# YoshuaNava/icpslam

Measured on AMD Instinct MI355X. Metric: icp_iterations_per_sec, higher is better.
Workload: dtype f32

## Files before the change

### icpslam_amd/csrc/icp_grid.hip

```cpp
#include <math.h>

#include <cstdlib>
#include <cstring>

#include "icp_env.h"
#include "icp_device.h"
#include "icp_grid_device.h"
#include "icp_kernels.h"

namespace icpgpu {
namespace {

__device__ __forceinline__ int enc_float(float f) {
  const int i = __float_as_int(f);
  return i >= 0 ? i : i ^ 0x7FFFFFFF;
}
inline float dec_float(int e) {
  const int i = e >= 0 ? e : e ^ 0x7FFFFFFF;
  float f;
  std::memcpy(&f, &i, 4);
  return f;
}

__global__ void bbox_init_kernel(int* mm) {
  if (threadIdx.x < 3) mm[threadIdx.x] = 0x7FFFFFFF;
  else if (threadIdx.x < 6) mm[threadIdx.x] = (int)0x80000000;
}

__global__ __launch_bounds__(256) void bbox_kernel(const float4* __restrict__ pts, int n, int* __restrict__ mm) {
  int lo[3] = {0x7FFFFFFF, 0x7FFFFFFF, 0x7FFFFFFF}, hi[3] = {(int)0x80000000, (int)0x80000000, (int)0x80000000};
  for (int i = blockIdx.x * 256 + threadIdx.x; i < n; i += gridDim.x * 256) {
    const float4 p = pts[i];
    if (finite3(p.x, p.y, p.z)) {
      const int e[3] = {enc_float(p.x), enc_float(p.y), enc_float(p.z)};
#pragma unroll
      for (int a = 0; a < 3; ++a) {
        lo[a] = min(lo[a], e[a]);
        hi[a] = max(hi[a], e[a]);
      }
    }
  }
#pragma unroll
  for (int a = 0; a < 3; ++a) {
#pragma unroll
    for (int off = 32; off > 0; off >>= 1) {
      lo[a] = min(lo[a], __shfl_down(lo[a], off, 64));
      hi[a] = max(hi[a], __shfl_down(hi[a], off, 64));
    }
  }
  __shared__ int wmm[4][6];
  const int lane = threadIdx.x & 63, wave = threadIdx.x >> 6;
  if (lane == 0) {
#pragma unroll
    for (int a = 0; a < 3; ++a) {
// ... 113 lines not shown
  int base = 0, total = 0;
#pragma unroll
  for (int w = 0; w < 16; ++w) {
    if (w < wave) base += wtot[w];
    total += wtot[w];
  }
  if (threadIdx.x == 0) stats[0] = total;
  int run = base + incl - s;
  for (int k = lo; k < hi; ++k) {
    const int v = block_sums[k];
    block_sums[k] = run;
    run += v;
  }
}

__global__ __launch_bounds__(256) void scan_apply_kernel(int* __restrict__ counts, int n, const int* __restrict__ block_sums,
                                                         const int* __restrict__ stats) {
  const int base = blockIdx.x * kScanItems + threadIdx.x * SCAN_PER_THREAD;
  int v[SCAN_PER_THREAD], s = 0;
#pragma unroll
  for (int k = 0; k < SCAN_PER_THREAD; ++k) {
    v[k] = (base + k < n) ? counts[base + k] : 0;
    s += v[k];
  }
  int tot;
  int run = block_exclusive_scan_256(s, &tot) + block_sums[blockIdx.x];
#pragma unroll
  for (int k = 0; k < SCAN_PER_THREAD; ++k) {
    if (base + k < n) counts[base + k] = run;
    run += v[k];
  }
  if (blockIdx.x == 0 && threadIdx.x == 0) counts[n] = stats[0];
}

__global__ __launch_bounds__(256) void grid_scatter_kernel(const float4* __restrict__ pts, int n,
                                                           const int* __restrict__ cell_of_point,
                                                           const int* __restrict__ rank,
                                                           const int* __restrict__ cell_start,
                                                           const int* __restrict__ orig_index,
                                                           float4* __restrict__ sorted) {
  const int i = blockIdx.x * 256 + threadIdx.x;
  if (i >= n) return;
  const int c = cell_of_point[i];
  if (c < 0) return;
  const float4 p = pts[i];
  sorted[cell_start[c] + rank[i]] = make_float4(p.x, p.y, p.z, __int_as_float(orig_index ? orig_index[i] : i));
}

constexpr int WQ_MAX_QPW = 16;

constexpr int WQ_WAVES = 4;
constexpr int WQ_BLOCK = WQ_WAVES * 64;

template <bool WRITE_KEYS, bool FUSE_REDUCE, bool LIST_UNMATCHED, bool PACK_SHORT_ROWS>
__global__ __launch_bounds__(WQ_BLOCK) void nn_wave_kernel(const float4* __restrict__ src, int n_s, int qpw, int xcd_map, Xform T,
                                                           const float4* __restrict__ sorted,
                                                           const int* __restrict__ cell_start, GridDesc g, float accept_thr,
                                                           unsigned long long* __restrict__ keys,
                                                           double* __restrict__ partials, int* __restrict__ unmatched,
                                                           int* __restrict__ unmatched_count) {
  const int lane = threadIdx.x & 63, wave = threadIdx.x >> 6;
  const int lb = xcd_map ? (int)(blockIdx.x & 7u) * (int)(gridDim.x >> 3) + (int)(blockIdx.x >> 3) : (int)blockIdx.x;
  const int k0 = lb * WQ_WAVES + wave, stride = gridDim.x * WQ_WAVES;

  double acc = 0.0;
  int qi = -1, pi = -1;
  if (lane >= 1 && lane <= 3) pi = lane - 1;
  else if (lane >= 4 && lane <= 6) qi = lane - 4;
  else if (lane >= 7 && lane <= 15) { qi = (lane - 7) / 3; pi = (lane - 7) % 3; }
  else if (lane == 16) qi = 3;

  float lpx = 0.f, lpy = 0.f, lpz = 0.f, lmargin = 0.5f;
  int lcx = 0, lcy = 0, lcz = 0, llo = 0, llen = 0;
  bool lfin = false;
  {
    const int sub = lane >> 2, il = k0 + sub * stride;
    if (sub < qpw && il < n_s) {
      const float4 s = src[il];
      xform_point(T, s.x, s.y, s.z, lpx, lpy, lpz);
      lfin = finite3(lpx, lpy, lpz);
      if (lfin) {
        cell_of(g, lpx, lpy, lpz, lcx, lcy, lcz);
        octant_row(cell_start, g, lpx, lpy, lpz, lcx, lcy, lcz, lane & 3, llo, llen, lmargin);
      }
    }
  }
  const unsigned long long fin_mask = __ballot(lfin), row_mask = __ballot(llen > 0);
  const float lsafe = lmargin * g.h * kGridSafety, lsafe_sq = lsafe * lsafe;
  unsigned long long my_key = kEmptyKey;

  for (int qq = 0; qq < qpw; ++qq) {
    const int i = k0 + qq * stride, l0 = qq * 4;
    if (i >= n_s) break;
    LaneBest b{kEmptyKey, 0.f, 0.f, 0.f};
    bool found = false;
    const float px = readlane_f(lpx, l0), py = readlane_f(lpy, l0), pz = readlane_f(lpz, l0);
    if ((fin_mask >> l0) & 1ull) {
      sweep_rows(sorted, llo, llen, row_mask & (0xFull << l0), lane, px, py, pz, b);
      found = merge_lanes(b) && __uint_as_float((unsigned int)(b.key >> 32)) <= readlane_f(lsafe_sq, l0);
      if (!found) {
        const int cx = __builtin_amdgcn_readlane(lcx, l0), cy = __builtin_amdgcn_readlane(lcy, l0),
                  cz = __builtin_amdgcn_readlane(lcz, l0);
        found = grow_cubes<PACK_SHORT_ROWS>(sorted, cell_start, g, px, py, pz, cx, cy, cz, lane, b);
      }
    }
    if constexpr (WRITE_KEYS) {
      if (lane == qq) my_key = found ? b.key : kEmptyKey;
    }
    if constexpr (LIST_UNMATCHED) {
      if (!found && lane == 0) unmatched[atomicAdd(unmatched_count, 1)] = i;
    }
    if constexpr (FUSE_REDUCE) {
      const float d2 = __uint_as_float((unsigned int)(b.key >> 32));
      if (found && d2 <= accept_thr) {
        const double a = qi < 0 ? 1.0 : (qi == 0 ? (double)b.qx : qi == 1 ? (double)b.qy : qi == 2 ? (double)b.qz : (double)d2);
        const double c = pi < 0 ? 1.0 : (pi == 0 ? (double)px : pi == 1 ? (double)py : (double)pz);
        acc += a * c;
      }
    }
  }
  if constexpr (WRITE_KEYS) {
    if (lane < qpw && k0 + lane * stride < n_s) keys[k0 + lane * stride] = my_key;
  }
  if constexpr (FUSE_REDUCE) {
    __shared__ double wterm[WQ_WAVES][kReduceTerms];
    if (lane < kReduceTerms) wterm[wave][lane] = acc;
    __syncthreads();
    if (threadIdx.x < kReduceTerms) {
      double v = 0.0;
#pragma unroll
      for (int w = 0; w < WQ_WAVES; ++w) v += wterm[w][threadIdx.x];
      partials[(size_t)threadIdx.x * gridDim.x + blockIdx.x] = v;
    }
  }
}

template <bool WRITE_KEYS, bool FUSE_REDUCE, bool LIST_UNMATCHED, bool PACK_SHORT_ROWS>
__device__ __forceinline__ void nn_quad_body(const float4* __restrict__ src, int n_s, int qpw, int xcd_map, const Xform& T,
                                             const float4* __restrict__ sorted, const int* __restrict__ cell_start,
                                             const GridDesc& g, float accept_thr, unsigned long long* __restrict__ keys,
                                             double* __restrict__ partials, int* __restrict__ unmatched,
                                             int* __restrict__ unmatched_count, unsigned int* __restrict__ prev_nn, int use_prev,
                                             int cube_start, unsigned long long* __restrict__ count_candidates, int n_blocks,
                                             int bx) {
  const int lane = threadIdx.x & 63, wave = threadIdx.x >> 6;
  const int grp_base = lane & 48, sub = lane & 15;
  unsigned int n_cand = 0;
  const int lb = xcd_map ? (bx & 7) * (n_blocks >> 3) + (bx >> 3) : bx;
  const int k0 = lb * WQ_WAVES + wave, stride = n_blocks * WQ_WAVES;

  double acc = 0.0;
  int cnt = 0;
  int qi = -1, pi = -1;
  if (sub == 0) qi = 3;
  else if (sub <= 3) pi = sub - 1;
  else if (sub <= 6) qi = sub - 4;
  else { qi = (sub - 7) / 3; pi = (sub - 7) % 3; }

  float lpx = 0.f, lpy = 0.f, lpz = 0.f, lmargin = 0.5f;
  int lcx = 0, lcy = 0, lcz = 0, llo = 0, llen = 0;
  bool lfin = false;
  const int il = k0 + (lane >> 2) * stride;
  const bool lvalid = (lane >> 2) < qpw && il < n_s;
  const char* __restrict__ sorted_bytes = reinterpret_cast<const char*>(sorted);
  float lbound = __builtin_nanf("");
  if (lvalid) {
    const float4 s = src[il];
    unsigned int ppos = kNoPrev;
    if (use_prev & 1) ppos = prev_nn[il];
    xform_point(T, s.x, s.y, s.z, lpx, lpy, lpz);
    lfin = finite3(lpx, lpy, lpz);
    if (lfin) {
      cell_of(g, lpx, lpy, lpz, lcx, lcy, lcz);
      if (ppos != kNoPrev) {
        const float4 pq = *reinterpret_cast<const float4*>(sorted_bytes + (size_t)ppos);
        lbound = dist2(pq.x, pq.y, pq.z, lpx, lpy, lpz);
      }
      octant_row_in_ball(cell_start, g, lpx, lpy, lpz, lcx, lcy, lcz, lane & 3, ball_cells_sq(g, lbound), llo, llen, lmargin);
    }
  }
  const unsigned long long fin_mask = __ballot(lfin);
  const float lsafe = lmargin * g.h * kGridSafety, lsafe_sq = lsafe * lsafe;
  const int n_pass = (__popcll(__ballot(lvalid)) + 15) >> 4;

  int slot_of_rank;
  {
    int cand = llen + __builtin_amdgcn_mov_dpp(llen, 0xB1, 0xF, 0xF, true);
    cand += __builtin_amdgcn_mov_dpp(cand, 0x4E, 0xF, 0xF, true);
    const unsigned int mine = ((lvalid ? (unsigned int)cand + 1u : 0u) << 4) | (unsigned int)(lane >> 2);
    int rank = 0;
#pragma unroll
    for (int k = 0; k < 16; ++k) rank += (unsigned int)__builtin_amdgcn_readlane((int)mine, 4 * k) > mine ? 1 : 0;
    slot_of_rank = __builtin_amdgcn_ds_permute((4 * rank + (lane & 3)) << 2, lane >> 2);
  }

  for (int pass = 0; pass < n_pass; ++pass) {
    const int ql = 4 * lane_get_i(slot_of_rank, 4 * (4 * pass + (lane >> 4)));
    const int qi_src = k0 + (ql >> 2) * stride;
    const bool valid = (ql >> 2) < qpw && qi_src < n_s;
    const float px = lane_get_f(lpx, ql), py = lane_get_f(lpy, ql), pz = lane_get_f(lpz, ql);
    const bool fin = (fin_mask >> ql) & 1ull;
    const int lo0 = lane_get_i(llo, ql), lo1 = lane_get_i(llo, ql + 1), lo2 = lane_get_i(llo, ql + 2), lo3 = lane_get_i(llo, ql + 3);
    const int n0 = lane_get_i(llen, ql), n1 = lane_get_i(llen, ql + 1), n2 = lane_get_i(llen, ql + 2), n3 = lane_get_i(llen, ql + 3);
    const int e0 = n0, e1 = e0 + n1, e2 = e1 + n2, L = e2 + n3;
    const unsigned int eb0 = (unsigned int)e0 << 4, eb1 = (unsigned int)e1 << 4, eb2 = (unsigned int)e2 << 4;
    const unsigned int ob0 = (unsigned int)lo0 << 4, ob1 = (unsigned int)(lo1 - e0) << 4, ob2 = (unsigned int)(lo2 - e1) << 4,
                       ob3 = L ? (unsigned int)(lo3 - e2) << 4 : 0u;
    const unsigned int lastb = (unsigned int)max(L - 1, 0) << 4;
    const int l_max = max(max(__builtin_amdgcn_readlane(L, 0), __builtin_amdgcn_readlane(L, 16)),
                          max(__builtin_amdgcn_readlane(L, 32), __builtin_amdgcn_readlane(L, 48)));
    if (count_candidates)
      n_cand += (unsigned int)(__builtin_amdgcn_readlane(L, 0) + __builtin_amdgcn_readlane(L, 16) + __builtin_amdgcn_readlane(L, 32) +
                               __builtin_amdgcn_readlane(L, 48));
    unsigned long long bkey = kEmptyKey;
    unsigned int bpos = 0u;
    unsigned int vb = (unsigned int)sub << 4;
    for (int done = 0; done < l_max; done += 32, vb += 512u) {
      const unsigned int ua = min(vb, lastb), ub = min(vb + 256u, lastb);
      const unsigned int fa = ua + (ua < eb0 ? ob0 : ua < eb1 ? ob1 : ua < eb2 ? ob2 : ob3);
      const unsigned int fb = ub + (ub < eb0 ? ob0 : ub < eb1 ? ob1 : ub < eb2 ? ob2 : ob3);
      const float4 qa = *reinterpret_cast<const float4*>(sorted_bytes + (size_t)fa);
      const float4 qb = *reinterpret_cast<const float4*>(sorted_bytes + (size_t)fb);
      __builtin_amdgcn_sched_barrier(0);
      const unsigned long long ka = ((unsigned long long)__float_as_uint(dist2(qa.x, qa.y, qa.z, px, py, pz)) << 32) | __float_as_uint(qa.w);
      const unsigned long long kb = ((unsigned long long)__float_as_uint(dist2(qb.x, qb.y, qb.z, px, py, pz)) << 32) | __float_as_uint(qb.w);
      if (ka < bkey) { bkey = ka; bpos = fa; }
      if (kb < bkey) { bkey = kb; bpos = fb; }
    }
    const unsigned int dbits = (unsigned int)(bkey >> 32), idx = (unsigned int)bkey;
    const unsigned int dmin = row16_min_u32(dbits);
    const unsigned int imin = row16_min_u32(dbits == dmin ? idx : 0xFFFFFFFFu);
    const unsigned long long win = __ballot(dbits == dmin && idx == imin);
    const int owner = grp_base + __ffs((unsigned int)(win >> grp_base) & 0xFFFFu) - 1;
    unsigned long long gkey = ((unsigned long long)dmin << 32) | imin;
    unsigned int wpos = (unsigned int)lane_get_i((int)bpos, owner);
    bool found = fin && __uint_as_float(dmin) <= lane_get_f(lsafe_sq, ql);

    unsigned long long need = (use_prev & 2) ? 0ull : __ballot(fin && !found && sub == 0);
    while (need) {
      const int gl = __ffsll((long long)need) - 1, sl = __builtin_amdgcn_readlane(ql, gl);
      need &= need - 1;
      const float ux = readlane_f(lpx, sl), uy = readlane_f(lpy, sl), uz = readlane_f(lpz, sl);
      const int cx = __builtin_amdgcn_readlane(lcx, sl), cy = __builtin_amdgcn_readlane(lcy, sl),
                cz = __builtin_amdgcn_readlane(lcz, sl);
      LanePos c{((unsigned long long)(unsigned int)__builtin_amdgcn_readlane((int)(gkey >> 32), gl) << 32) |
                    (unsigned int)__builtin_amdgcn_readlane((int)gkey, gl),
                (unsigned int)__builtin_amdgcn_readlane((int)wpos, gl)};
      const float pb = readlane_f(lbound, sl);
      if (pb < __builtin_inff() && !(__uint_as_float((unsigned int)(c.key >> 32)) <= pb)) {
        c.key = ((unsigned long long)__float_as_uint(pb) << 32) | 0xFFFFFFFFull;
        c.pos = prev_nn[k0 + (sl >> 2) * stride];
      }
      int rho_first = 1;
      {
        const float seed = __uint_as_float((unsigned int)(c.key >> 32));
        const int cap = (use_prev & 1) ? ((cube_start & 1) ? g.r_max : 1) : min((cube_start >> 8) & 0xFF, g.r_max);
        if (seed < __builtin_inff() && cap > 1)
          rho_first = max(1, min((int)ceilf(__builtin_amdgcn_sqrtf(seed) * g.inv_h * (1.0f / kGridSafety)), cap));
      }
      const bool f2 = grow_cubes<PACK_SHORT_ROWS>(sorted, cell_start, g, ux, uy, uz, cx, cy, cz, lane, c, rho_first,
                                                  count_candidates ? &n_cand : nullptr);
      if (grp_base == gl) {
        gkey = c.key;
        wpos = c.pos;
        found = f2;
      }
    }

    if (prev_nn && sub == 0 && valid) {
      const float bd = __uint_as_float((unsigned int)(gkey >> 32));
      prev_nn[qi_src] = (fin && bd == bd) ? wpos : kNoPrev;
    }
    if constexpr (WRITE_KEYS) {
      if (sub == 0 && valid) keys[qi_src] = found ? gkey : kEmptyKey;
    }
    if constexpr (LIST_UNMATCHED) {
      if (sub == 0 && valid && !found) unmatched[atomicAdd(unmatched_count, 1)] = qi_src;
    }
    if constexpr (FUSE_REDUCE) {
      const float d2 = __uint_as_float((unsigned int)(gkey >> 32));
      if (found && d2 <= accept_thr) {
        const float4 w = *reinterpret_cast<const float4*>(sorted_bytes + (size_t)wpos);
        const float qx = w.x, qy = w.y, qz = w.z;
        const float af = qi == 0 ? qx : qi == 1 ? qy : qi == 2 ? qz : qi == 3 ? d2 : 1.0f;
        const float cf = pi == 0 ? px : pi == 1 ? py : pi == 2 ? pz : 1.0f;
        acc += (double)af * (double)cf;
        cnt += 1;
      }
    }
  }
  if (count_candidates && lane == 0) atomicAdd(count_candidates, (unsigned long long)n_cand);
  if constexpr (FUSE_REDUCE) {
    __shared__ double wterm[WQ_WAVES * 4][16];
    __shared__ int wcnt[WQ_WAVES * 4];
    wterm[wave * 4 + (lane >> 4)][sub] = acc;
    if (sub == 0) wcnt[wave * 4 + (lane >> 4)] = cnt;
    __syncthreads();
    if (threadIdx.x < kReduceTerms) {
      double v = 0.0;
      if (threadIdx.x == 0) {
        int n = 0;
#pragma unroll
        for (int k = 0; k < WQ_WAVES * 4; ++k) n += wcnt[k];
        v = (double)n;
      } else {
        const int s = threadIdx.x == 16 ? 0 : (int)threadIdx.x;
#pragma unroll
        for (int k = 0; k < WQ_WAVES * 4; ++k) v += wterm[k][s];
      }
      partials[(size_t)threadIdx.x * n_blocks + bx] = v;
    }
  }
}


template <bool WRITE_KEYS, bool FUSE_REDUCE, bool LIST_UNMATCHED, bool PACK_SHORT_ROWS>
__global__ __launch_bounds__(WQ_BLOCK) __attribute__((amdgpu_waves_per_eu(8, 8))) void nn_quad_kernel(const float4* __restrict__ src, int n_s, int qpw, int xcd_map, Xform T,
                                                           const float4* __restrict__ sorted,
                                                           const int* __restrict__ cell_start, GridDesc g, float accept_thr,
                                                           unsigned long long* __restrict__ keys,
                                                           double* __restrict__ partials, int* __restrict__ unmatched,
                                                           int* __restrict__ unmatched_count, unsigned int* __restrict__ prev_nn,
                                                           int use_prev, int cube_start,
                                                           unsigned long long* __restrict__ count_candidates) {
  nn_quad_body<WRITE_KEYS, FUSE_REDUCE, LIST_UNMATCHED, PACK_SHORT_ROWS>(src, n_s, qpw, xcd_map, T, sorted, cell_start, g, accept_thr, keys,
                                                                        partials, unmatched, unmatched_count, prev_nn, use_prev,
                                                                        cube_start, count_candidates, (int)gridDim.x, (int)blockIdx.x);
}

template <bool PACK_SHORT_ROWS, bool OPEN>
__global__ __launch_bounds__(WQ_BLOCK) __attribute__((amdgpu_waves_per_eu(8, 8))) void nn_quad_batch_kernel(const BatchPair* __restrict__ pairs, BatchStep step,
                                                                                                       int cube_start) {
  const int by = (int)blockIdx.y, bx = (int)blockIdx.x;
  const BatchPair& d = pairs[step.slot[by]];
  const int n_blocks = d.blocks;
  if (bx >= n_blocks) return;
  const Xform T = step.T[by];
  GridDesc g = d.g;
  const int use_prev = (int)((step.use_prev_mask >> by) & 1u);
  if constexpr (OPEN) {
    g.r_max = d.r_max_open;
    nn_quad_body<true, false, true, PACK_SHORT_ROWS>(d.src, d.n_s, d.qpw, d.xcd_map, T, d.sorted, d.cell_start, g, 0.f, d.keys, nullptr,
                                                     d.unmatched, d.unmatched_count, d.prev_nn, use_prev, cube_start, nullptr, n_blocks, bx);
  } else {
    nn_quad_body<false, true, false, PACK_SHORT_ROWS>(d.src, d.n_s, d.qpw, d.xcd_map, T, d.sorted, d.cell_start, g, d.accept_thr, nullptr,
                                                      d.partials, nullptr, nullptr, d.prev_nn, use_prev, cube_start, nullptr, n_blocks, bx);
  }
}

}

hipError_t launch_bbox(const float4* pts, int n, int* d_minmax6, hipStream_t stream, bool init) {
  if (init) hipLaunchKernelGGL(bbox_init_kernel, dim3(1), dim3(64), 0, stream, d_minmax6);
  if (n > 0) {
    int blocks = (n + 255) / 256;
    if (blocks > 256) blocks = 256;
    hipLaunchKernelGGL(bbox_kernel, dim3(blocks), dim3(256), 0, stream, pts, n, d_minmax6);
  }
  return hipGetLastError();
}

void decode_bbox(const int enc[6], float lo[3], float hi[3]) {
  for (int a = 0; a < 3; ++a) {
    lo[a] = dec_float(enc[a]);
    hi[a] = dec_float(enc[3 + a]);
  }
}

hipError_t launch_grid_count(const float4* pts, int n, const GridDesc& g, int* cell_of_point, int* rank_in_cell,
                             int* counts, int* block_sums, int* d_stats, hipStream_t stream) {
  const int ncells = g.nx * g.ny * g.nz;
  {
    const size_t n_counts = (size_t)ncells + 1;
    const size_t want = (n_counts / 4 + 255) / 256;
    const int blocks = (int)(want < 1 ? 1 : want > 4096 ? 4096 : want);
    hipLaunchKernelGGL(grid_clear_kernel, dim3(blocks), dim3(256), 0, stream, counts, n_counts, d_stats);
  }
  if (n > 0)
    hipLaunchKernelGGL(grid_count_kernel, dim3((n + 255) / 256), dim3(256), 0, stream, pts, n, g, cell_of_point,
                       rank_in_cell, counts);
  const int nb = (ncells + kScanItems - 1) / kScanItems;
  hipLaunchKernelGGL(scan_sums_kernel, dim3(nb), dim3(256), 0, stream, counts, ncells, block_sums, d_stats);
  return hipGetLastError();
}

hipError_t launch_grid_finish(const float4* pts, int n, const GridDesc& g, const int* cell_of_point,
                              const int* rank_in_cell, int* counts, int* block_sums, int* d_stats, const int* orig_index,
                              float4* sorted, hipStream_t stream) {
  const int ncells = g.nx * g.ny * g.nz;
  const int nb = (ncells + kScanItems - 1) / kScanItems;
  hipLaunchKernelGGL(scan_top_kernel, dim3(1), dim3(1024), 0, stream, block_sums, nb, d_stats);
  hipLaunchKernelGGL(scan_apply_kernel, dim3(nb), dim3(256), 0, stream, counts, ncells, block_sums, d_stats);
  if (n > 0)
    hipLaunchKernelGGL(grid_scatter_kernel, dim3((n + 255) / 256), dim3(256), 0, stream, pts, n, cell_of_point,
                       rank_in_cell, counts, orig_index, sorted);
  return hipGetLastError();
}

static bool quad_enabled() {
  static const bool v = [] { const char* e = ICPGPU_DEV_ENV("ICPGPU_QUAD"); return !e || atoi(e) != 0; }();
  return v;
}
static unsigned long long* g_count_candidates = nullptr;
static int quad_debug_bits() {
  static const int v = [] {
    if (!ICPGPU_DEV_ENV("ICPGPU_SKIP_UNCERT")) return 0;
    fprintf(stderr, "[icpgpu] WARNING: ICPGPU_SKIP_UNCERT is set -- uncertified points are DROPPED, every result of this process is WRONG "
                    "(a timing experiment's switch, never a production setting)\n");
    return 2;
  }();
  return v;
}
static int cube_start_mask() {
  static const int v = [] {
    const char* e = ICPGPU_DEV_ENV("ICPGPU_CUBE_START");
    const char* c = ICPGPU_DEV_ENV("ICPGPU_CUBE_COLD_CAP");
    const int warm = e ? (atoi(e) & 1) : 1, cold = c ? atoi(c) : 1;
    return warm | ((cold < 1 ? 1 : cold > 255 ? 255 : cold) << 8);
  }();
  return v;
}
static bool use_quad(int n_s) { return quad_enabled() && n_s >= 4 * 8192; }

static int queries_per_wave(int n_s) {
  static const int forced = [] { const char* e = ICPGPU_DEV_ENV("ICPGPU_QPW"); return e ? atoi(e) : 0; }();
  if (forced >= 4 && forced <= WQ_MAX_QPW && use_quad(n_s)) return forced & ~3;
  int q = n_s / 8192;
  if (use_quad(n_s)) q = (q + 3) & ~3;
  if (q < 1) q = 1;
  if (q > WQ_MAX_QPW) q = WQ_MAX_QPW;
  return q;
}

void grid_count_candidates(unsigned long long* device_counter) { g_count_candidates = device_counter; }

bool grid_search_batchable(int n_s, int flags) { return use_quad(n_s) && !(flags & kGridOver4GiB) && queries_per_wave(n_s) > 0; }
int grid_search_qpw(int n_s) { return queries_per_wave(n_s); }

hipError_t launch_nn_grid_search_batch(const BatchPair* d_pairs, const BatchStep& step, int n_active, int max_blocks, bool pack,
                                       bool open_range, hipStream_t stream) {
  if (n_active <= 0 || max_blocks <= 0) return hipSuccess;
  const dim3 grid((unsigned)max_blocks, (unsigned)n_active), block(WQ_BLOCK);
  if (pack && open_range) hipLaunchKernelGGL((nn_quad_batch_kernel<true, true>), grid, block, 0, stream, d_pairs, step, cube_start_mask());
  else if (pack) hipLaunchKernelGGL((nn_quad_batch_kernel<true, false>), grid, block, 0, stream, d_pairs, step, cube_start_mask());
  else if (open_range) hipLaunchKernelGGL((nn_quad_batch_kernel<false, true>), grid, block, 0, stream, d_pairs, step, cube_start_mask());
  else hipLaunchKernelGGL((nn_quad_batch_kernel<false, false>), grid, block, 0, stream, d_pairs, step, cube_start_mask());
  return hipGetLastError();
}

bool grid_search_keeps_prev(int n_s, int flags) { return use_quad(n_s) && !(flags & kGridOver4GiB); }

int grid_search_blocks(int n_s) {
  const int per_block = WQ_WAVES * queries_per_wave(n_s);
  const int nb = (n_s + per_block - 1) / per_block;
  return (nb + 7) & ~7;
}

hipError_t launch_nn_grid_search(const float4* src, int n_s, int flags, const Xform& T, const float4* sorted,
                                 const int* cell_start, const GridDesc& g, float accept_thr, unsigned long long* keys,
                                 double* partials, int* unmatched, int* unmatched_count, hipStream_t stream,
                                 unsigned int* prev_nn, bool use_prev) {
  if (n_s <= 0) return hipSuccess;
  const int blocks = grid_search_blocks(n_s);
  const int qpw = queries_per_wave(n_s), xm = flags & kGridSrcInCellOrder;
  const bool pack = (flags & kGridPackShortRows) != 0;
  dim3 grid(blocks), block(WQ_BLOCK);
  const bool quad = use_quad(n_s) && !(flags & kGridOver4GiB);
#define ICP_LAUNCH_WQP(K, F, U, P)                                                                                      \
  do {                                                                                                                  \
    if (quad)                                                                                                           \
      hipLaunchKernelGGL((nn_quad_kernel<K, F, U, P>), grid, block, 0, stream, src, n_s, qpw, xm, T, sorted, cell_start, \
                         g, accept_thr, keys, partials, unmatched, unmatched_count, prev_nn,                    \
                         ((prev_nn && use_prev) ? 1 : 0) | quad_debug_bits(), cube_start_mask(), g_count_candidates);     \
    else                                                                                                                \
      hipLaunchKernelGGL((nn_wave_kernel<K, F, U, P>), grid, block, 0, stream, src, n_s, qpw, xm, T, sorted, cell_start, \
                         g, accept_thr, keys, partials, unmatched, unmatched_count);                                    \
  } while (0)
#define ICP_LAUNCH_WQ(K, F, U)              \
  do {                                      \
    if (pack) ICP_LAUNCH_WQP(K, F, U, true); \
    else ICP_LAUNCH_WQP(K, F, U, false);     \
  } while (0)
  const bool k = keys != nullptr, f = partials != nullptr, u = unmatched != nullptr;
  if (k && !f && u) ICP_LAUNCH_WQ(true, false, true);
  else if (k && !f) ICP_LAUNCH_WQ(true, false, false);
  else if (!k && f && !u) ICP_LAUNCH_WQ(false, true, false);
  else if (k && f && !u) ICP_LAUNCH_WQ(true, true, false);
  else return hipErrorInvalidValue;
#undef ICP_LAUNCH_WQP
#undef ICP_LAUNCH_WQ
  return hipGetLastError();
}

}
```

Before: 13690.

## Add persistent batch loop to grid NN search sized by device occupancy

Adds a BATCHES template path where each wave loops over several 16-query batches, so a grid sized to the resident wave count covers all source points. The change also sizes queries-per-wave from the occupancy API (per-CU blocks times CU count) instead of a hardcoded constant. The batch loop is only compiled under a developer switch, so by default only the occupancy-based qpw sizing changes. The aim is to cut launch tail effects and fit the grid to the device, at the cost of more template instantiations and host-side occupancy queries.

```diff
diff --git a/icpslam_amd/csrc/icp_grid.hip b/icpslam_amd/csrc/icp_grid.hip
--- a/icpslam_amd/csrc/icp_grid.hip
+++ b/icpslam_amd/csrc/icp_grid.hip
@@ -1,5 +1,7 @@
 #include <math.h>
 
+#include <atomic>
+#include <cstdio>
 #include <cstdlib>
 #include <cstring>
 
@@ -219,7 +221,7 @@
 constexpr int WQ_WAVES = 4;
 constexpr int WQ_BLOCK = WQ_WAVES * 64;
 
-template <bool WRITE_KEYS, bool FUSE_REDUCE, bool LIST_UNMATCHED, bool PACK_SHORT_ROWS>
+template <bool WRITE_KEYS, bool FUSE_REDUCE, bool LIST_UNMATCHED, bool PACK_SHORT_ROWS, bool BATCHES>
 __global__ __launch_bounds__(WQ_BLOCK) void nn_wave_kernel(const float4* __restrict__ src, int n_s, int qpw, int xcd_map, Xform T,
                                                            const float4* __restrict__ sorted,
                                                            const int* __restrict__ cell_start, GridDesc g, float accept_thr,
@@ -237,57 +239,62 @@
   else if (lane >= 7 && lane <= 15) { qi = (lane - 7) / 3; pi = (lane - 7) % 3; }
   else if (lane == 16) qi = 3;
 
-  float lpx = 0.f, lpy = 0.f, lpz = 0.f, lmargin = 0.5f;
-  int lcx = 0, lcy = 0, lcz = 0, llo = 0, llen = 0;
-  bool lfin = false;
-  {
-    const int sub = lane >> 2, il = k0 + sub * stride;
-    if (sub < qpw && il < n_s) {
-      const float4 s = src[il];
-      xform_point(T, s.x, s.y, s.z, lpx, lpy, lpz);
-      lfin = finite3(lpx, lpy, lpz);
-      if (lfin) {
-        cell_of(g, lpx, lpy, lpz, lcx, lcy, lcz);
-        octant_row(cell_start, g, lpx, lpy, lpz, lcx, lcy, lcz, lane & 3, llo, llen, lmargin);
-      }
-    }
-  }
-  const unsigned long long fin_mask = __ballot(lfin), row_mask = __ballot(llen > 0);
-  const float lsafe = lmargin * g.h * kGridSafety, lsafe_sq = lsafe * lsafe;
-  unsigned long long my_key = kEmptyKey;
-
-  for (int qq = 0; qq < qpw; ++qq) {
-    const int i = k0 + qq * stride, l0 = qq * 4;
-    if (i >= n_s) break;
-    LaneBest b{kEmptyKey, 0.f, 0.f, 0.f};
-    bool found = false;
-    const float px = readlane_f(lpx, l0), py = readlane_f(lpy, l0), pz = readlane_f(lpz, l0);
-    if ((fin_mask >> l0) & 1ull) {
-      sweep_rows(sorted, llo, llen, row_mask & (0xFull << l0), lane, px, py, pz, b);
-      found = merge_lanes(b) && __uint_as_float((unsigned int)(b.key >> 32)) <= readlane_f(lsafe_sq, l0);
-      if (!found) {
-        const int cx = __builtin_amdgcn_readlane(lcx, l0), cy = __builtin_amdgcn_readlane(lcy, l0),
-                  cz = __builtin_amdgcn_readlane(lcz, l0);
-        found = grow_cubes<PACK_SHORT_ROWS>(sorted, cell_start, g, px, py, pz, cx, cy, cz, lane, b);
+  const int batch_stride = 16 * stride;
+  for (int kb = k0; !BATCHES || kb < n_s;) {
+    float lpx = 0.f, lpy = 0.f, lpz = 0.f, lmargin = 0.5f;
+    int lcx = 0, lcy = 0, lcz = 0, llo = 0, llen = 0;
+    bool lfin = false;
+    {
+      const int sub = lane >> 2, il = kb + sub * stride;
+      if (sub < qpw && il < n_s) {
+        const float4 s = src[il];
+        xform_point(T, s.x, s.y, s.z, lpx, lpy, lpz);
+        lfin = finite3(lpx, lpy, lpz);
+        if (lfin) {
+          cell_of(g, lpx, lpy, lpz, lcx, lcy, lcz);
+          octant_row(cell_start, g, lpx, lpy, lpz, lcx, lcy, lcz, lane & 3, llo, llen, lmargin);
+        }
+      }
+    }
+    const unsigned long long fin_mask = __ballot(lfin), row_mask = __ballot(llen > 0);
+    const float lsafe = lmargin * g.h * kGridSafety, lsafe_sq = lsafe * lsafe;
+    unsigned long long my_key = kEmptyKey;
+
+    for (int qq = 0; qq < qpw; ++qq) {
+      const int i = kb + qq * stride, l0 = qq * 4;
+      if (i >= n_s) break;
+      LaneBest b{kEmptyKey, 0.f, 0.f, 0.f};
+      bool found = false;
+      const float px = readlane_f(lpx, l0), py = readlane_f(lpy, l0), pz = readlane_f(lpz, l0);
+      if ((fin_mask >> l0) & 1ull) {
+        sweep_rows(sorted, llo, llen, row_mask & (0xFull << l0), lane, px, py, pz, b);
+        found = merge_lanes(b) && __uint_as_float((unsigned int)(b.key >> 32)) <= readlane_f(lsafe_sq, l0);
+        if (!found) {
+          const int cx = __builtin_amdgcn_readlane(lcx, l0), cy = __builtin_amdgcn_readlane(lcy, l0),
+                    cz = __builtin_amdgcn_readlane(lcz, l0);
+          found = grow_cubes<PACK_SHORT_ROWS>(sorted, cell_start, g, px, py, pz, cx, cy, cz, lane, b);
+        }
+      }
+      if constexpr (WRITE_KEYS) {
+        if (lane == qq) my_key = found ? b.key : kEmptyKey;
+      }
+      if constexpr (LIST_UNMATCHED) {
+        if (!found && lane == 0) unmatched[atomicAdd(unmatched_count, 1)] = i;
+      }
+      if constexpr (FUSE_REDUCE) {
+        const float d2 = __uint_as_float((unsigned int)(b.key >> 32));
+        if (found && d2 <= accept_thr) {
+          const double a = qi < 0 ? 1.0 : (qi == 0 ? (double)b.qx : qi == 1 ? (double)b.qy : qi == 2 ? (double)b.qz : (double)d2);
+          const double c = pi < 0 ? 1.0 : (pi == 0 ? (double)px : pi == 1 ? (double)py : (double)pz);
+          acc += a * c;
+        }
       }
     }
     if constexpr (WRITE_KEYS) {
-      if (lane == qq) my_key = found ? b.key : kEmptyKey;
-    }
-    if constexpr (LIST_UNMATCHED) {
-      if (!found && lane == 0) unmatched[atomicAdd(unmatched_count, 1)] = i;
-    }
-    if constexpr (FUSE_REDUCE) {
-      const float d2 = __uint_as_float((unsigned int)(b.key >> 32));
-      if (found && d2 <= accept_thr) {
-        const double a = qi < 0 ? 1.0 : (qi == 0 ? (double)b.qx : qi == 1 ? (double)b.qy : qi == 2 ? (double)b.qz : (double)d2);
-        const double c = pi < 0 ? 1.0 : (pi == 0 ? (double)px : pi == 1 ? (double)py : (double)pz);
-        acc += a * c;
-      }
-    }
-  }
-  if constexpr (WRITE_KEYS) {
-    if (lane < qpw && k0 + lane * stride < n_s) keys[k0 + lane * stride] = my_key;
+      if (lane < qpw && kb + lane * stride < n_s) keys[kb + lane * stride] = my_key;
+    }
+    if (!BATCHES || n_s - kb <= batch_stride) break;
+    kb += batch_stride;
   }
   if constexpr (FUSE_REDUCE) {
     __shared__ double wterm[WQ_WAVES][kReduceTerms];
@@ -302,7 +309,7 @@
   }
 }
 
-template <bool WRITE_KEYS, bool FUSE_REDUCE, bool LIST_UNMATCHED, bool PACK_SHORT_ROWS>
+template <bool WRITE_KEYS, bool FUSE_REDUCE, bool LIST_UNMATCHED, bool PACK_SHORT_ROWS, bool BATCHES>
 __device__ __forceinline__ void nn_quad_body(const float4* __restrict__ src, int n_s, int qpw, int xcd_map, const Xform& T,
                                              const float4* __restrict__ sorted, const int* __restrict__ cell_start,
                                              const GridDesc& g, float accept_thr, unsigned long long* __restrict__ keys,
@@ -324,137 +331,142 @@
   else if (sub <= 6) qi = sub - 4;
   else { qi = (sub - 7) / 3; pi = (sub - 7) % 3; }
 
-  float lpx = 0.f, lpy = 0.f, lpz = 0.f, lmargin = 0.5f;
-  int lcx = 0, lcy = 0, lcz = 0, llo = 0, llen = 0;
-  bool lfin = false;
-  const int il = k0 + (lane >> 2) * stride;
-  const bool lvalid = (lane >> 2) < qpw && il < n_s;
-  const char* __restrict__ sorted_bytes = reinterpret_cast<const char*>(sorted);
-  float lbound = __builtin_nanf("");
-  if (lvalid) {
-    const float4 s = src[il];
-    unsigned int ppos = kNoPrev;
-    if (use_prev & 1) ppos = prev_nn[il];
-    xform_point(T, s.x, s.y, s.z, lpx, lpy, lpz);
-    lfin = finite3(lpx, lpy, lpz);
-    if (lfin) {
-      cell_of(g, lpx, lpy, lpz, lcx, lcy, lcz);
-      if (ppos != kNoPrev) {
-        const float4 pq = *reinterpret_cast<const float4*>(sorted_bytes + (size_t)ppos);
-        lbound = dist2(pq.x, pq.y, pq.z, lpx, lpy, lpz);
-      }
-      octant_row_in_ball(cell_start, g, lpx, lpy, lpz, lcx, lcy, lcz, lane & 3, ball_cells_sq(g, lbound), llo, llen, lmargin);
-    }
-  }
-  const unsigned long long fin_mask = __ballot(lfin);
-  const float lsafe = lmargin * g.h * kGridSafety, lsafe_sq = lsafe * lsafe;
-  const int n_pass = (__popcll(__ballot(lvalid)) + 15) >> 4;
-
-  int slot_of_rank;
-  {
-    int cand = llen + __builtin_amdgcn_mov_dpp(llen, 0xB1, 0xF, 0xF, true);
-    cand += __builtin_amdgcn_mov_dpp(cand, 0x4E, 0xF, 0xF, true);
-    const unsigned int mine = ((lvalid ? (unsigned int)cand + 1u : 0u) << 4) | (unsigned int)(lane >> 2);
-    int rank = 0;
-#pragma unroll
-    for (int k = 0; k < 16; ++k) rank += (unsigned int)__builtin_amdgcn_readlane((int)mine, 4 * k) > mine ? 1 : 0;
-    slot_of_rank = __builtin_amdgcn_ds_permute((4 * rank + (lane & 3)) << 2, lane >> 2);
-  }
-
-  for (int pass = 0; pass < n_pass; ++pass) {
-    const int ql = 4 * lane_get_i(slot_of_rank, 4 * (4 * pass + (lane >> 4)));
-    const int qi_src = k0 + (ql >> 2) * stride;
-    const bool valid = (ql >> 2) < qpw && qi_src < n_s;
-    const float px = lane_get_f(lpx, ql), py = lane_get_f(lpy, ql), pz = lane_get_f(lpz, ql);
-    const bool fin = (fin_mask >> ql) & 1ull;
-    const int lo0 = lane_get_i(llo, ql), lo1 = lane_get_i(llo, ql + 1), lo2 = lane_get_i(llo, ql + 2), lo3 = lane_get_i(llo, ql + 3);
-    const int n0 = lane_get_i(llen, ql), n1 = lane_get_i(llen, ql + 1), n2 = lane_get_i(llen, ql + 2), n3 = lane_get_i(llen, ql + 3);
-    const int e0 = n0, e1 = e0 + n1, e2 = e1 + n2, L = e2 + n3;
-    const unsigned int eb0 = (unsigned int)e0 << 4, eb1 = (unsigned int)e1 << 4, eb2 = (unsigned int)e2 << 4;
-    const unsigned int ob0 = (unsigned int)lo0 << 4, ob1 = (unsigned int)(lo1 - e0) << 4, ob2 = (unsigned int)(lo2 - e1) << 4,
-                       ob3 = L ? (unsigned int)(lo3 - e2) << 4 : 0u;
-    const unsigned int lastb = (unsigned int)max(L - 1, 0) << 4;
-    const int l_max = max(max(__builtin_amdgcn_readlane(L, 0), __builtin_amdgcn_readlane(L, 16)),
-                          max(__builtin_amdgcn_readlane(L, 32), __builtin_amdgcn_readlane(L, 48)));
-    if (count_candidates)
-      n_cand += (unsigned int)(__builtin_amdgcn_readlane(L, 0) + __builtin_amdgcn_readlane(L, 16) + __builtin_amdgcn_readlane(L, 32) +
-                               __builtin_amdgcn_readlane(L, 48));
-    unsigned long long bkey = kEmptyKey;
-    unsigned int bpos = 0u;
-    unsigned int vb = (unsigned int)sub << 4;
-    for (int done = 0; done < l_max; done += 32, vb += 512u) {
-      const unsigned int ua = min(vb, lastb), ub = min(vb + 256u, lastb);
-      const unsigned int fa = ua + (ua < eb0 ? ob0 : ua < eb1 ? ob1 : ua < eb2 ? ob2 : ob3);
-      const unsigned int fb = ub + (ub < eb0 ? ob0 : ub < eb1 ? ob1 : ub < eb2 ? ob2 : ob3);
-      const float4 qa = *reinterpret_cast<const float4*>(sorted_bytes + (size_t)fa);
-      const float4 qb = *reinterpret_cast<const float4*>(sorted_bytes + (size_t)fb);
-      __builtin_amdgcn_sched_barrier(0);
-      const unsigned long long ka = ((unsigned long long)__float_as_uint(dist2(qa.x, qa.y, qa.z, px, py, pz)) << 32) | __float_as_uint(qa.w);
-      const unsigned long long kb = ((unsigned long long)__float_as_uint(dist2(qb.x, qb.y, qb.z, px, py, pz)) << 32) | __float_as_uint(qb.w);
-      if (ka < bkey) { bkey = ka; bpos = fa; }
-      if (kb < bkey) { bkey = kb; bpos = fb; }
-    }
-    const unsigned int dbits = (unsigned int)(bkey >> 32), idx = (unsigned int)bkey;
-    const unsigned int dmin = row16_min_u32(dbits);
-    const unsigned int imin = row16_min_u32(dbits == dmin ? idx : 0xFFFFFFFFu);
-    const unsigned long long win = __ballot(dbits == dmin && idx == imin);
-    const int owner = grp_base + __ffs((unsigned int)(win >> grp_base) & 0xFFFFu) - 1;
-    unsigned long long gkey = ((unsigned long long)dmin << 32) | imin;
-    unsigned int wpos = (unsigned int)lane_get_i((int)bpos, owner);
-    bool found = fin && __uint_as_float(dmin) <= lane_get_f(lsafe_sq, ql);
-
-    unsigned long long need = (use_prev & 2) ? 0ull : __ballot(fin && !found && sub == 0);
-    while (need) {
-      const int gl = __ffsll((long long)need) - 1, sl = __builtin_amdgcn_readlane(ql, gl);
-      need &= need - 1;
-      const float ux = readlane_f(lpx, sl), uy = readlane_f(lpy, sl), uz = readlane_f(lpz, sl);
-      const int cx = __builtin_amdgcn_readlane(lcx, sl), cy = __builtin_amdgcn_readlane(lcy, sl),
-                cz = __builtin_amdgcn_readlane(lcz, sl);
-      LanePos c{((unsigned long long)(unsigned int)__builtin_amdgcn_readlane((int)(gkey >> 32), gl) << 32) |
-                    (unsigned int)__builtin_amdgcn_readlane((int)gkey, gl),
-                (unsigned int)__builtin_amdgcn_readlane((int)wpos, gl)};
-      const float pb = readlane_f(lbound, sl);
-      if (pb < __builtin_inff() && !(__uint_as_float((unsigned int)(c.key >> 32)) <= pb)) {
-        c.key = ((unsigned long long)__float_as_uint(pb) << 32) | 0xFFFFFFFFull;
-        c.pos = prev_nn[k0 + (sl >> 2) * stride];
-      }
-      int rho_first = 1;
-      {
-        const float seed = __uint_as_float((unsigned int)(c.key >> 32));
-        const int cap = (use_prev & 1) ? ((cube_start & 1) ? g.r_max : 1) : min((cube_start >> 8) & 0xFF, g.r_max);
-        if (seed < __builtin_inff() && cap > 1)
-          rho_first = max(1, min((int)ceilf(__builtin_amdgcn_sqrtf(seed) * g.inv_h * (1.0f / kGridSafety)), cap));
-      }
-      const bool f2 = grow_cubes<PACK_SHORT_ROWS>(sorted, cell_start, g, ux, uy, uz, cx, cy, cz, lane, c, rho_first,
-                                                  count_candidates ? &n_cand : nullptr);
-      if (grp_base == gl) {
-        gkey = c.key;
-        wpos = c.pos;
-        found = f2;
-      }
-    }
-
-    if (prev_nn && sub == 0 && valid) {
-      const float bd = __uint_as_float((unsigned int)(gkey >> 32));
-      prev_nn[qi_src] = (fin && bd == bd) ? wpos : kNoPrev;
-    }
-    if constexpr (WRITE_KEYS) {
-      if (sub == 0 && valid) keys[qi_src] = found ? gkey : kEmptyKey;
-    }
-    if constexpr (LIST_UNMATCHED) {
-      if (sub == 0 && valid && !found) unmatched[atomicAdd(unmatched_count, 1)] = qi_src;
-    }
-    if constexpr (FUSE_REDUCE) {
-      const float d2 = __uint_as_float((unsigned int)(gkey >> 32));
-      if (found && d2 <= accept_thr) {
-        const float4 w = *reinterpret_cast<const float4*>(sorted_bytes + (size_t)wpos);
-        const float qx = w.x, qy = w.y, qz = w.z;
-        const float af = qi == 0 ? qx : qi == 1 ? qy : qi == 2 ? qz : qi == 3 ? d2 : 1.0f;
-        const float cf = pi == 0 ? px : pi == 1 ? py : pi == 2 ? pz : 1.0f;
-        acc += (double)af * (double)cf;
-        cnt += 1;
-      }
-    }
+  const int batch_stride = 16 * stride;
+  for (int kb = k0; !BATCHES || kb < n_s;) {
+    float lpx = 0.f, lpy = 0.f, lpz = 0.f, lmargin = 0.5f;
+    int lcx = 0, lcy = 0, lcz = 0, llo = 0, llen = 0;
+    bool lfin = false;
+    const int il = kb + (lane >> 2) * stride;
+    const bool lvalid = (lane >> 2) < qpw && il < n_s;
+    const char* __restrict__ sorted_bytes = reinterpret_cast<const char*>(sorted);
+    float lbound = __builtin_nanf("");
+    if (lvalid) {
+      const float4 s = src[il];
+      unsigned int ppos = kNoPrev;
+      if (use_prev & 1) ppos = prev_nn[il];
+      xform_point(T, s.x, s.y, s.z, lpx, lpy, lpz);
+      lfin = finite3(lpx, lpy, lpz);
+      if (lfin) {
+        cell_of(g, lpx, lpy, lpz, lcx, lcy, lcz);
+        if (ppos != kNoPrev) {
+          const float4 pq = *reinterpret_cast<const float4*>(sorted_bytes + (size_t)ppos);
+          lbound = dist2(pq.x, pq.y, pq.z, lpx, lpy, lpz);
+        }
+        octant_row_in_ball(cell_start, g, lpx, lpy, lpz, lcx, lcy, lcz, lane & 3, ball_cells_sq(g, lbound), llo, llen, lmargin);
+      }
+    }
+    const unsigned long long fin_mask = __ballot(lfin);
+    const float lsafe = lmargin * g.h * kGridSafety, lsafe_sq = lsafe * lsafe;
+    const int n_pass = (__popcll(__ballot(lvalid)) + 15) >> 4;
+
+    int slot_of_rank;
+    {
+      int cand = llen + __builtin_amdgcn_mov_dpp(llen, 0xB1, 0xF, 0xF, true);
+      cand += __builtin_amdgcn_mov_dpp(cand, 0x4E, 0xF, 0xF, true);
+      const unsigned int mine = ((lvalid ? (unsigned int)cand + 1u : 0u) << 4) | (unsigned int)(lane >> 2);
+      int rank = 0;
+  #pragma unroll
+      for (int k = 0; k < 16; ++k) rank += (unsigned int)__builtin_amdgcn_readlane((int)mine, 4 * k) > mine ? 1 : 0;
+      slot_of_rank = __builtin_amdgcn_ds_permute((4 * rank + (lane & 3)) << 2, lane >> 2);
+    }
+
+    for (int pass = 0; pass < n_pass; ++pass) {
+      const int ql = 4 * lane_get_i(slot_of_rank, 4 * (4 * pass + (lane >> 4)));
+      const int qi_src = kb + (ql >> 2) * stride;
+      const bool valid = (ql >> 2) < qpw && qi_src < n_s;
+      const float px = lane_get_f(lpx, ql), py = lane_get_f(lpy, ql), pz = lane_get_f(lpz, ql);
+      const bool fin = (fin_mask >> ql) & 1ull;
+      const int lo0 = lane_get_i(llo, ql), lo1 = lane_get_i(llo, ql + 1), lo2 = lane_get_i(llo, ql + 2), lo3 = lane_get_i(llo, ql + 3);
+      const int n0 = lane_get_i(llen, ql), n1 = lane_get_i(llen, ql + 1), n2 = lane_get_i(llen, ql + 2), n3 = lane_get_i(llen, ql + 3);
+      const int e0 = n0, e1 = e0 + n1, e2 = e1 + n2, L = e2 + n3;
+      const unsigned int eb0 = (unsigned int)e0 << 4, eb1 = (unsigned int)e1 << 4, eb2 = (unsigned int)e2 << 4;
+      const unsigned int ob0 = (unsigned int)lo0 << 4, ob1 = (unsigned int)(lo1 - e0) << 4, ob2 = (unsigned int)(lo2 - e1) << 4,
+                         ob3 = L ? (unsigned int)(lo3 - e2) << 4 : 0u;
+      const unsigned int lastb = (unsigned int)max(L - 1, 0) << 4;
+      const int l_max = max(max(__builtin_amdgcn_readlane(L, 0), __builtin_amdgcn_readlane(L, 16)),
+                            max(__builtin_amdgcn_readlane(L, 32), __builtin_amdgcn_readlane(L, 48)));
+      if (count_candidates)
+        n_cand += (unsigned int)(__builtin_amdgcn_readlane(L, 0) + __builtin_amdgcn_readlane(L, 16) + __builtin_amdgcn_readlane(L, 32) +
+                                 __builtin_amdgcn_readlane(L, 48));
+      unsigned long long bkey = kEmptyKey;
+      unsigned int bpos = 0u;
+      unsigned int vb = (unsigned int)sub << 4;
+      for (int done = 0; done < l_max; done += 32, vb += 512u) {
+        const unsigned int ua = min(vb, lastb), ub = min(vb + 256u, lastb);
+        const unsigned int fa = ua + (ua < eb0 ? ob0 : ua < eb1 ? ob1 : ua < eb2 ? ob2 : ob3);
+        const unsigned int fb = ub + (ub < eb0 ? ob0 : ub < eb1 ? ob1 : ub < eb2 ? ob2 : ob3);
+        const float4 qa = *reinterpret_cast<const float4*>(sorted_bytes + (size_t)fa);
+        const float4 qb = *reinterpret_cast<const float4*>(sorted_bytes + (size_t)fb);
+        __builtin_amdgcn_sched_barrier(0);
+        const unsigned long long ka = ((unsigned long long)__float_as_uint(dist2(qa.x, qa.y, qa.z, px, py, pz)) << 32) | __float_as_uint(qa.w);
+        const unsigned long long kb = ((unsigned long long)__float_as_uint(dist2(qb.x, qb.y, qb.z, px, py, pz)) << 32) | __float_as_uint(qb.w);
+        if (ka < bkey) { bkey = ka; bpos = fa; }
+        if (kb < bkey) { bkey = kb; bpos = fb; }
+      }
+      const unsigned int dbits = (unsigned int)(bkey >> 32), idx = (unsigned int)bkey;
+      const unsigned int dmin = row16_min_u32(dbits);
+      const unsigned int imin = row16_min_u32(dbits == dmin ? idx : 0xFFFFFFFFu);
+      const unsigned long long win = __ballot(dbits == dmin && idx == imin);
+      const int owner = grp_base + __ffs((unsigned int)(win >> grp_base) & 0xFFFFu) - 1;
+      unsigned long long gkey = ((unsigned long long)dmin << 32) | imin;
+      unsigned int wpos = (unsigned int)lane_get_i((int)bpos, owner);
+      bool found = fin && __uint_as_float(dmin) <= lane_get_f(lsafe_sq, ql);
+
+      unsigned long long need = (use_prev & 2) ? 0ull : __ballot(fin && !found && sub == 0);
+      while (need) {
+        const int gl = __ffsll((long long)need) - 1, sl = __builtin_amdgcn_readlane(ql, gl);
+        need &= need - 1;
+        const float ux = readlane_f(lpx, sl), uy = readlane_f(lpy, sl), uz = readlane_f(lpz, sl);
+        const int cx = __builtin_amdgcn_readlane(lcx, sl), cy = __builtin_amdgcn_readlane(lcy, sl),
+                  cz = __builtin_amdgcn_readlane(lcz, sl);
+        LanePos c{((unsigned long long)(unsigned int)__builtin_amdgcn_readlane((int)(gkey >> 32), gl) << 32) |
+                      (unsigned int)__builtin_amdgcn_readlane((int)gkey, gl),
+                  (unsigned int)__builtin_amdgcn_readlane((int)wpos, gl)};
+        const float pb = readlane_f(lbound, sl);
+        if (pb < __builtin_inff() && !(__uint_as_float((unsigned int)(c.key >> 32)) <= pb)) {
+          c.key = ((unsigned long long)__float_as_uint(pb) << 32) | 0xFFFFFFFFull;
+          c.pos = prev_nn[kb + (sl >> 2) * stride];
+        }
+        int rho_first = 1;
+        {
+          const float seed = __uint_as_float((unsigned int)(c.key >> 32));
+          const int cap = (use_prev & 1) ? ((cube_start & 1) ? g.r_max : 1) : min((cube_start >> 8) & 0xFF, g.r_max);
+          if (seed < __builtin_inff() && cap > 1)
+            rho_first = max(1, min((int)ceilf(__builtin_amdgcn_sqrtf(seed) * g.inv_h * (1.0f / kGridSafety)), cap));
+        }
+        const bool f2 = grow_cubes<PACK_SHORT_ROWS>(sorted, cell_start, g, ux, uy, uz, cx, cy, cz, lane, c, rho_first,
+                                                    count_candidates ? &n_cand : nullptr);
+        if (grp_base == gl) {
+          gkey = c.key;
+          wpos = c.pos;
+          found = f2;
+        }
+      }
+
+      if (prev_nn && sub == 0 && valid) {
+        const float bd = __uint_as_float((unsigned int)(gkey >> 32));
+        prev_nn[qi_src] = (fin && bd == bd) ? wpos : kNoPrev;
+      }
+      if constexpr (WRITE_KEYS) {
+        if (sub == 0 && valid) keys[qi_src] = found ? gkey : kEmptyKey;
+      }
+      if constexpr (LIST_UNMATCHED) {
+        if (sub == 0 && valid && !found) unmatched[atomicAdd(unmatched_count, 1)] = qi_src;
+      }
+      if constexpr (FUSE_REDUCE) {
+        const float d2 = __uint_as_float((unsigned int)(gkey >> 32));
+        if (found && d2 <= accept_thr) {
+          const float4 w = *reinterpret_cast<const float4*>(sorted_bytes + (size_t)wpos);
+          const float qx = w.x, qy = w.y, qz = w.z;
+          const float af = qi == 0 ? qx : qi == 1 ? qy : qi == 2 ? qz : qi == 3 ? d2 : 1.0f;
+          const float cf = pi == 0 ? px : pi == 1 ? py : pi == 2 ? pz : 1.0f;
+          acc += (double)af * (double)cf;
+          cnt += 1;
+        }
+      }
+    }
+    if (!BATCHES || n_s - kb <= batch_stride) break;
+    kb += batch_stride;
   }
   if (count_candidates && lane == 0) atomicAdd(count_candidates, (unsigned long long)n_cand);
   if constexpr (FUSE_REDUCE) {
@@ -481,7 +493,7 @@
 }
 
 
-template <bool WRITE_KEYS, bool FUSE_REDUCE, bool LIST_UNMATCHED, bool PACK_SHORT_ROWS>
+template <bool WRITE_KEYS, bool FUSE_REDUCE, bool LIST_UNMATCHED, bool PACK_SHORT_ROWS, bool BATCHES>
 __global__ __launch_bounds__(WQ_BLOCK) __attribute__((amdgpu_waves_per_eu(8, 8))) void nn_quad_kernel(const float4* __restrict__ src, int n_s, int qpw, int xcd_map, Xform T,
                                                            const float4* __restrict__ sorted,
                                                            const int* __restrict__ cell_start, GridDesc g, float accept_thr,
@@ -490,12 +502,12 @@
                                                            int* __restrict__ unmatched_count, unsigned int* __restrict__ prev_nn,
                                                            int use_prev, int cube_start,
                                                            unsigned long long* __restrict__ count_candidates) {
-  nn_quad_body<WRITE_KEYS, FUSE_REDUCE, LIST_UNMATCHED, PACK_SHORT_ROWS>(src, n_s, qpw, xcd_map, T, sorted, cell_start, g, accept_thr, keys,
+  nn_quad_body<WRITE_KEYS, FUSE_REDUCE, LIST_UNMATCHED, PACK_SHORT_ROWS, BATCHES>(src, n_s, qpw, xcd_map, T, sorted, cell_start, g, accept_thr, keys,
                                                                         partials, unmatched, unmatched_count, prev_nn, use_prev,
                                                                         cube_start, count_candidates, (int)gridDim.x, (int)blockIdx.x);
 }
 
-template <bool PACK_SHORT_ROWS, bool OPEN>
+template <bool PACK_SHORT_ROWS, bool OPEN, bool BATCHES>
 __global__ __launch_bounds__(WQ_BLOCK) __attribute__((amdgpu_waves_per_eu(8, 8))) void nn_quad_batch_kernel(const BatchPair* __restrict__ pairs, BatchStep step,
                                                                                                        int cube_start) {
   const int by = (int)blockIdx.y, bx = (int)blockIdx.x;
@@ -507,10 +519,10 @@
   const int use_prev = (int)((step.use_prev_mask >> by) & 1u);
   if constexpr (OPEN) {
     g.r_max = d.r_max_open;
-    nn_quad_body<true, false, true, PACK_SHORT_ROWS>(d.src, d.n_s, d.qpw, d.xcd_map, T, d.sorted, d.cell_start, g, 0.f, d.keys, nullptr,
+    nn_quad_body<true, false, true, PACK_SHORT_ROWS, BATCHES>(d.src, d.n_s, d.qpw, d.xcd_map, T, d.sorted, d.cell_start, g, 0.f, d.keys, nullptr,
                                                      d.unmatched, d.unmatched_count, d.prev_nn, use_prev, cube_start, nullptr, n_blocks, bx);
   } else {
-    nn_quad_body<false, true, false, PACK_SHORT_ROWS>(d.src, d.n_s, d.qpw, d.xcd_map, T, d.sorted, d.cell_start, g, d.accept_thr, nullptr,
+    nn_quad_body<false, true, false, PACK_SHORT_ROWS, BATCHES>(d.src, d.n_s, d.qpw, d.xcd_map, T, d.sorted, d.cell_start, g, d.accept_thr, nullptr,
                                                       d.partials, nullptr, nullptr, d.prev_nn, use_prev, cube_start, nullptr, n_blocks, bx);
   }
 }
@@ -587,18 +599,65 @@
   }();
   return v;
 }
-static bool use_quad(int n_s) { return quad_enabled() && n_s >= 4 * 8192; }
-
-static int queries_per_wave(int n_s) {
-  static const int forced = [] { const char* e = ICPGPU_DEV_ENV("ICPGPU_QPW"); return e ? atoi(e) : 0; }();
-  if (forced >= 4 && forced <= WQ_MAX_QPW && use_quad(n_s)) return forced & ~3;
-  int q = n_s / 8192;
+constexpr int kQuadMinPoints = 32768;
+static bool use_quad(int n_s) { return quad_enabled() && n_s >= kQuadMinPoints; }
+
+static int device_resident_waves() {
+  constexpr int kMaxDevices = 64;
+  static std::atomic<int> cache[kMaxDevices];
+  int dev = 0;
+  if (hipGetDevice(&dev) != hipSuccess || dev < 0 || dev >= kMaxDevices) return 0;
+  int v = cache[dev].load(std::memory_order_relaxed);
+  if (v == 0) {
+    int per_cu = 0, cus = 0;
+    const hipError_t e1 = hipOccupancyMaxActiveBlocksPerMultiprocessor(&per_cu, nn_quad_kernel<false, true, false, false, false>, WQ_BLOCK, 0);
+    const hipError_t e2 = hipDeviceGetAttribute(&cus, hipDeviceAttributeMultiprocessorCount, dev);
+    v = (e1 == hipSuccess && e2 == hipSuccess && per_cu > 0 && cus > 0) ? per_cu * cus * WQ_WAVES : -1;
+    if (v < 0)
+      fprintf(stderr, "[icpgpu] device %d: no occupancy figure for the grid search (%s / %s); an MI355X's is assumed\n", dev,
+              hipGetErrorString(e1), hipGetErrorString(e2));
+    cache[dev].store(v, std::memory_order_relaxed);
+  }
+  return v > 0 ? v : 0;
+}
+#if defined(ICPGPU_DEV_SWITCHES)
+constexpr bool kBatchLoopBuilt = true;
+#else
+constexpr bool kBatchLoopBuilt = false;
+#endif
+static int resident_waves() {
+  if (!kBatchLoopBuilt) return 0;
+  static const int forced = [] { const char* e = ICPGPU_DEV_ENV("ICPGPU_RESIDENT_WAVES"); return e ? atoi(e) : 0; }();
+  return forced >= 0 ? forced : device_resident_waves();
+}
+
+static int forced_qpw() {
+  static const int v = [] { const char* e = ICPGPU_DEV_ENV("ICPGPU_QPW"); return e ? atoi(e) : 0; }();
+  return (v >= 4 && v <= WQ_MAX_QPW) ? (v & ~3) : 0;
+}
+constexpr int kResidentWavesMI355X = 256 * 4 * 8;
+static int queries_per_wave_one_batch(int n_s) {
+  if (forced_qpw() && use_quad(n_s)) return forced_qpw();
+  const int slots = device_resident_waves();
+  int q = n_s / (slots > 0 ? slots : kResidentWavesMI355X);
   if (use_quad(n_s)) q = (q + 3) & ~3;
   if (q < 1) q = 1;
   if (q > WQ_MAX_QPW) q = WQ_MAX_QPW;
   return q;
 }
 
+struct SearchGeometry {
+  int qpw, blocks;
+};
+static SearchGeometry search_geometry(int n_s) {
+  const int waves = (resident_waves() / (8 * WQ_WAVES)) * (8 * WQ_WAVES);
+  if (waves > 0 && !(forced_qpw() && use_quad(n_s)) && (long long)n_s > 19ll * waves) return {WQ_MAX_QPW, waves / WQ_WAVES};
+  const int qpw = queries_per_wave_one_batch(n_s), per_block = WQ_WAVES * qpw;
+  const int nb = (n_s + per_block - 1) / per_block;
+  return {qpw, (nb + 7) & ~7};
+}
+static int queries_per_wave(int n_s) { return search_geometry(n_s).qpw; }
+
 void grid_count_candidates(unsigned long long* device_counter) { g_count_candidates = device_counter; }
 
 bool grid_search_batchable(int n_s, int flags) { return use_quad(n_s) && !(flags & kGridOver4GiB) && queries_per_wave(n_s) > 0; }
@@ -608,41 +667,56 @@
                                        bool open_range, hipStream_t stream) {
   if (n_active <= 0 || max_blocks <= 0) return hipSuccess;
   const dim3 grid((unsigned)max_blocks, (unsigned)n_active), block(WQ_BLOCK);
-  if (pack && open_range) hipLaunchKernelGGL((nn_quad_batch_kernel<true, true>), grid, block, 0, stream, d_pairs, step, cube_start_mask());
-  else if (pack) hipLaunchKernelGGL((nn_quad_batch_kernel<true, false>), grid, block, 0, stream, d_pairs, step, cube_start_mask());
-  else if (open_range) hipLaunchKernelGGL((nn_quad_batch_kernel<false, true>), grid, block, 0, stream, d_pairs, step, cube_start_mask());
-  else hipLaunchKernelGGL((nn_quad_batch_kernel<false, false>), grid, block, 0, stream, d_pairs, step, cube_start_mask());
+#define ICP_LAUNCH_BATCH(B)                                                                                                              \
+  do {                                                                                                                                   \
+    if (pack && open_range) hipLaunchKernelGGL((nn_quad_batch_kernel<true, true, B>), grid, block, 0, stream, d_pairs, step, cube_start_mask());   \
+    else if (pack) hipLaunchKernelGGL((nn_quad_batch_kernel<true, false, B>), grid, block, 0, stream, d_pairs, step, cube_start_mask());           \
+    else if (open_range) hipLaunchKernelGGL((nn_quad_batch_kernel<false, true, B>), grid, block, 0, stream, d_pairs, step, cube_start_mask());     \
+    else hipLaunchKernelGGL((nn_quad_batch_kernel<false, false, B>), grid, block, 0, stream, d_pairs, step, cube_start_mask());                    \
+  } while (0)
+#if defined(ICPGPU_DEV_SWITCHES)
+  if (resident_waves() != 0) ICP_LAUNCH_BATCH(true);
+  else
+#endif
+    ICP_LAUNCH_BATCH(false);
+#undef ICP_LAUNCH_BATCH
   return hipGetLastError();
 }
 
 bool grid_search_keeps_prev(int n_s, int flags) { return use_quad(n_s) && !(flags & kGridOver4GiB); }
 
-int grid_search_blocks(int n_s) {
-  const int per_block = WQ_WAVES * queries_per_wave(n_s);
-  const int nb = (n_s + per_block - 1) / per_block;
-  return (nb + 7) & ~7;
-}
+int grid_search_blocks(int n_s) { return search_geometry(n_s).blocks; }
 
 hipError_t launch_nn_grid_search(const float4* src, int n_s, int flags, const Xform& T, const float4* sorted,
                                  const int* cell_start, const GridDesc& g, float accept_thr, unsigned long long* keys,
                                  double* partials, int* unmatched, int* unmatched_count, hipStream_t stream,
                                  unsigned int* prev_nn, bool use_prev) {
   if (n_s <= 0) return hipSuccess;
-  const int blocks = grid_search_blocks(n_s);
-  const int qpw = queries_per_wave(n_s), xm = flags & kGridSrcInCellOrder;
+  const SearchGeometry geo = search_geometry(n_s);
+  const int blocks = geo.blocks, qpw = geo.qpw, xm = flags & kGridSrcInCellOrder;
   const bool pack = (flags & kGridPackShortRows) != 0;
   dim3 grid(blocks), block(WQ_BLOCK);
   const bool quad = use_quad(n_s) && !(flags & kGridOver4GiB);
-#define ICP_LAUNCH_WQP(K, F, U, P)                                                                                      \
-  do {                                                                                                                  \
-    if (quad)                                                                                                           \
-      hipLaunchKernelGGL((nn_quad_kernel<K, F, U, P>), grid, block, 0, stream, src, n_s, qpw, xm, T, sorted, cell_start, \
-                         g, accept_thr, keys, partials, unmatched, unmatched_count, prev_nn,                    \
+#define ICP_LAUNCH_WQPB(K, F, U, P, B)                                                                                    \
+  do {                                                                                                                    \
+    if (quad)                                                                                                             \
+      hipLaunchKernelGGL((nn_quad_kernel<K, F, U, P, B>), grid, block, 0, stream, src, n_s, qpw, xm, T, sorted, cell_start, \
+                         g, accept_thr, keys, partials, unmatched, unmatched_count, prev_nn,                              \
                          ((prev_nn && use_prev) ? 1 : 0) | quad_debug_bits(), cube_start_mask(), g_count_candidates);     \
-    else                                                                                                                \
-      hipLaunchKernelGGL((nn_wave_kernel<K, F, U, P>), grid, block, 0, stream, src, n_s, qpw, xm, T, sorted, cell_start, \
-                         g, accept_thr, keys, partials, unmatched, unmatched_count);                                    \
+    else                                                                                                                  \
+      hipLaunchKernelGGL((nn_wave_kernel<K, F, U, P, B>), grid, block, 0, stream, src, n_s, qpw, xm, T, sorted,            \
+                         cell_start, g, accept_thr, keys, partials, unmatched, unmatched_count);                          \
   } while (0)
+#if defined(ICPGPU_DEV_SWITCHES)
+  const bool batches = resident_waves() != 0;
+#define ICP_LAUNCH_WQP(K, F, U, P)                  \
+  do {                                              \
+    if (batches) ICP_LAUNCH_WQPB(K, F, U, P, true);  \
+    else ICP_LAUNCH_WQPB(K, F, U, P, false);         \
+  } while (0)
+#else
+#define ICP_LAUNCH_WQP(K, F, U, P) ICP_LAUNCH_WQPB(K, F, U, P, false)
+#endif
 #define ICP_LAUNCH_WQ(K, F, U)              \
   do {                                      \
     if (pack) ICP_LAUNCH_WQP(K, F, U, true); \
@@ -654,6 +728,7 @@
   else if (!k && f && !u) ICP_LAUNCH_WQ(false, true, false);
   else if (k && f && !u) ICP_LAUNCH_WQ(true, true, false);
   else return hipErrorInvalidValue;
+#undef ICP_LAUNCH_WQPB
 #undef ICP_LAUNCH_WQP
 #undef ICP_LAUNCH_WQ
   return hipGetLastError();
```

Result: slower. 13390 (-2.2%).
